# ZhongLingXiao/nano-kazen

Hardware: NVIDIA B200
Metric: Mpaths/s (higher is better)
Workload: dtype f32

## Files before the change

nano-kazen_b200/csrc/kz_kernels.cuh:

```cuda
#ifndef KZ_KERNELS_CUH
#define KZ_KERNELS_CUH
#include "kz_path.h"

#ifndef KZ_TRACE_THREADS
#define KZ_TRACE_THREADS 128
#endif
#ifndef KZ_TRACE_MIN_BLOCKS
#define KZ_TRACE_MIN_BLOCKS 8
#endif
#ifndef KZ_BATCH_MIN_BLOCKS
#define KZ_BATCH_MIN_BLOCKS 8
#endif
#define KZ_SHADE_THREADS 128

struct KzControl {
    unsigned long long ext_shadow[2];
    uint32_t n_class[KZ_NUM_CLASSES];
    uint32_t head_ext, head_shadow, head_trace;
    uint32_t pad[1];
    unsigned long long paths, rays_ext, rays_shadow, vertices, rays_seeded;
};

struct KzQueues {
    uint32_t *ext[2];
    uint32_t *cls[KZ_NUM_CLASSES];
    uint32_t *shadow;
};

struct KzChunk {
    int32_t x0, y0, x1, y1;
    uint32_t tiles_x;
    uint32_t npx_padded;
    int32_t spp_begin;
    uint32_t n_spp;
    uint32_t spp_group;
    unsigned long long first;
    uint32_t count;
};

#define KZ_FULL 0xFFFFFFFFu

__device__ __forceinline__ uint32_t kz_lane() { return threadIdx.x & 31u; }

__device__ __forceinline__ void kz_push(uint32_t *queue, uint32_t *counter, bool pred, uint32_t value) {
// ... 37 lines not shown
        v += __shfl_down_sync(KZ_FULL, v, o);
        h += __shfl_down_sync(KZ_FULL, h, o);
    }
    if (kz_lane() == 0u) {
        if (e) atomicAdd(&ctl->rays_ext, e);
        if (s) atomicAdd(&ctl->rays_shadow, s);
        if (v) atomicAdd(&ctl->vertices, v);
        if (h) atomicAdd(&ctl->rays_seeded, h);
    }
}

struct KzRayIn { float ox, oy, oz, tmin, dx, dy, dz, tmax; };
#ifndef KZ_FETCH_ND
#define KZ_FETCH_ND 0
#endif
#ifndef KZ_FETCH_NW
#define KZ_FETCH_NW 8
#endif
#ifndef KZ_TRAV_MODE
#define KZ_TRAV_MODE 0
#endif
#ifndef KZ_WAIT_IDLE
#define KZ_WAIT_IDLE 1
#endif
#ifndef KZ_POSTPONE_NUM
#define KZ_POSTPONE_NUM 1
#define KZ_POSTPONE_DEN 5
#endif

template <class Job>
__device__ __forceinline__ void kz_warp_trace(const KzScene &sc, const KzStackRef &stk, uint32_t *cursor, uint32_t n, Job &job) {
    KzTrav t;
    KzLocalStack ls;
    t.sp = 0; t.ng_y = 0u; t.tg_y = 0u;
    bool active = false, finished = false, exhausted = false;
    uint32_t item = 0u;
    const uint32_t lane = kz_lane(), lt = (1u << lane) - 1u;
    for (;;) {
        if (finished) {
            KzRayIn r;
            if (job.end(item, t.best, r)) kz_trav_init(sc, t, r.ox, r.oy, r.oz, r.dx, r.dy, r.dz, r.tmin, r.tmax);
            else active = false;
            finished = false;
        }
        if (!exhausted) {
            const uint32_t idle = __ballot_sync(KZ_FULL, !active);
            if (idle) {
                const uint32_t leader = (uint32_t)__ffs((int)idle) - 1u;
                uint32_t base = 0u;
                if (lane == leader) base = atomicAdd(cursor, (uint32_t)__popc(idle));
                base = __shfl_sync(KZ_FULL, base, (int)leader);
                if (!active) {
                    const uint32_t idx = base + (uint32_t)__popc(idle & lt);
                    if (idx < n) {
                        item = idx;
                        KzRayIn r;
                        job.begin(item, r);
                        kz_trav_init(sc, t, r.ox, r.oy, r.oz, r.dx, r.dy, r.dz, r.tmin, r.tmax);
                        job.seed(sc, t);
                        active = true;
                    }
                }
                exhausted = base + (uint32_t)__popc(idle) >= n;
            }
        }
        if (!__any_sync(KZ_FULL, active)) break;
        int lost = 0;
#if KZ_TRAV_MODE == 1
        while (active && !finished) {
            for (;;) {
                if (t.ng_y > 0x00FFFFFFu) kz_trav_node(sc, t, stk, ls);
                if (t.tg_y != 0u) break;
                if (t.ng_y <= 0x00FFFFFFu) {
                    if (t.sp == 0) break;
                    kz_trav_pop(t, stk, ls);
                }
            }
            while (t.tg_y != 0u) kz_trav_tri(sc, t);
            if (t.ng_y <= 0x00FFFFFFu) {
                if (t.sp == 0) finished = true;
                else kz_trav_pop(t, stk, ls);
            }
            if (!exhausted) {
                lost += 32 - __popc(__activemask()) - KZ_FETCH_ND;
                if (lost >= KZ_FETCH_NW) break;
            }
        }
#else
        while (active && !finished) {
#if KZ_WAIT_IDLE
            if (t.tg_y == 0u && t.ng_y > 0x00FFFFFFu) kz_trav_node(sc, t, stk, ls);
            const int total = __popc(__activemask());
// ... 59 lines not shown
    }
}

__global__ void __launch_bounds__(KZ_SHADE_THREADS) k_raygen(KzScene sc, KzPathState st, uint32_t *q0, KzChunk ch) {
    const uint32_t i = blockIdx.x * blockDim.x + threadIdx.x;
    if (i >= ch.count) return;
    unsigned long long g = ch.first + i;
    const unsigned long long per_block = (unsigned long long)ch.npx_padded * ch.spp_group;
    const uint32_t blk = (uint32_t)(g / per_block);
    g -= (unsigned long long)blk * per_block;
    const uint32_t left = ch.n_spp - blk * ch.spp_group;
    const uint32_t grp = left < ch.spp_group ? left : ch.spp_group;
    const uint32_t tile = (uint32_t)(g / (32u * grp));
    const uint32_t r = (uint32_t)(g - (unsigned long long)tile * (32u * grp));
    const uint32_t s_local = blk * ch.spp_group + (r >> 5), in_tile = r & 31u;
    const int x = ch.x0 + (int)((tile % ch.tiles_x) * 8u + (in_tile & 7u));
    const int y = ch.y0 + (int)((tile / ch.tiles_x) * 4u + (in_tile >> 3));
    if (x < ch.x1 && y < ch.y1) kz_raygen_item(sc, st, i, x, y, (uint32_t)(ch.spp_begin + (int)s_local));
    else {
        const float nan = kz_u2f(0x7FC00000u);
        KzRayRec ray; ray.o = mkf4(0.f, 0.f, 0.f, 0.f); ray.d = mkf4(nan, nan, nan, 0.f);
        st.a[i].ray = ray;
        st.b[i].smp.pix = 0xFFFFFFFFu;
    }
    q0[i] = i;
}

template <bool FIRST>
struct KzExtendJob {
    static constexpr bool kStopsEarly = false;
    __device__ __forceinline__ bool stop(const KzScene &, const KzTrav &) { return false; }
    const KzScene &sc; const KzPathState &st; KzControl *ctl; const KzQueues &q; const uint32_t *queue;
    uint2 *hint;
    KzCounters cnt;
    uint32_t slot, n_seeded;
    KzHit first_hit; bool retraced;
    kz3 d;
    __device__ KzExtendJob(const KzScene &s, const KzPathState &p, KzControl *c, const KzQueues &qq, const uint32_t *qu, uint2 *h)
        : sc(s), st(p), ctl(c), q(qq), queue(qu), hint(h), n_seeded(0u) { cnt.paths = cnt.rays_ext = cnt.rays_shadow = cnt.vertices = cnt.rays_seeded = 0ull; }
    __device__ __forceinline__ size_t hint_index() const {
        const uint32_t pix = st.b[slot].smp.pix, px = pix & 0xFFFFu, py = pix >> 16;
        if (px >= (uint32_t)sc.camera.width || py >= (uint32_t)sc.camera.height) return ~(size_t)0;
        return (size_t)py * (uint32_t)sc.camera.width + px;
    }
    __device__ __forceinline__ void seed(const KzScene &s, KzTrav &t) {
        if (!FIRST || hint == nullptr) return;
        const size_t i = hint_index();
        if (i == ~(size_t)0) return;
        const uint2 h = hint[i];
        n_seeded += kz_trav_seed(s, t, h.x, h.y) ? 1u : 0u;
    }
    __device__ __forceinline__ void begin(uint32_t item, KzRayIn &r) {
        slot = queue[item];
        const KzRayRec ray = st.a[slot].ray;
        const KzF4 ro = ray.o, rd = ray.d;
        r.ox = ro.x; r.oy = ro.y; r.oz = ro.z; r.tmin = ro.w; r.dx = rd.x; r.dy = rd.y; r.dz = rd.z; r.tmax = rd.w;
        d = mk3(rd.x, rd.y, rd.z);
        retraced = false;
    }
    __device__ __forceinline__ bool end(uint32_t, const KzHit &hit, KzRayIn &r) {
        if (FIRST && isnan(d.x)) return false;
        cnt.rays_ext += 1;
        KzHit h = hit;
        if (FIRST) {
            if (hint != nullptr && !retraced) { const size_t i = hint_index(); if (i != ~(size_t)0) hint[i] = make_uint2(h.geom, h.prim); }
            if (retraced) { if (h.geom == KZ_INVALID_ID) h = first_hit; }
            else if (h.geom != KZ_INVALID_ID && sc.integrator.type == KZ_INTEGRATOR_PATH_MIS) {
                const uint32_t fl = sc.meshes[h.geom].flags;
                if ((fl & KZ_MESH_IS_LIGHT) && !(fl & KZ_MESH_LIGHT_VISIBLE)) {
                    KzIts its; its.acc_rough = 0.f;
                    fill_intersection(sc, h, its, mk3(0.f));
                    const kz3 o = its.p + sc.integrator.trace_bias * d;
                    r.ox = o.x; r.oy = o.y; r.oz = o.z; r.tmin = KZ_EPSILON; r.dx = d.x; r.dy = d.y; r.dz = d.z; r.tmax = KZ_INF;
                    first_hit = h; retraced = true;
                    return true;
                }
            }
        }
        st.a[slot].hit = mk_hit_rec(h);
        kz_push_divergent(q.cls, ctl->n_class, kz_classify(sc, h.geom), slot);
        return false;
    }
};

template <bool FIRST>
__global__ void __launch_bounds__(KZ_TRACE_THREADS, KZ_TRACE_MIN_BLOCKS) k_extend(KzScene sc, KzPathState st, KzControl *ctl, KzQueues q, int cur, uint2 *hint) {
    const KzStackRef stk = kz_trav_shared_init();
    KzExtendJob<FIRST> job(sc, st, ctl, q, q.ext[cur], FIRST ? hint : nullptr);
    kz_warp_trace(sc, stk, &ctl->head_ext, kz_ext_count(ctl, cur), job);
    job.cnt.rays_seeded = job.n_seeded;
    kz_flush_counters(ctl, job.cnt);
}

#ifndef KZ_SHADE_BLOCK_PUSH
#define KZ_SHADE_BLOCK_PUSH 1
#endif
#ifndef KZ_SHADE_MIN_BLOCKS_DIFFUSE
#define KZ_SHADE_MIN_BLOCKS_DIFFUSE 8
#endif
#ifndef KZ_SHADE_MIN_BLOCKS_TERMINAL
#define KZ_SHADE_MIN_BLOCKS_TERMINAL 4
#endif
#ifndef KZ_SHADE_MIN_BLOCKS
#define KZ_SHADE_MIN_BLOCKS 4
#endif
template <int CLS>
__global__ void __launch_bounds__(KZ_SHADE_THREADS, (CLS == KZ_CLASS_DIFFUSE ? KZ_SHADE_MIN_BLOCKS_DIFFUSE : (CLS == KZ_CLASS_TERMINAL ? KZ_SHADE_MIN_BLOCKS_TERMINAL : KZ_SHADE_MIN_BLOCKS))) k_shade(KzScene sc, KzPathState st, KzControl *ctl, KzQueues q, int nxt, int bounce) {
    const uint32_t n = ctl->n_class[CLS];
    const uint32_t *queue = q.cls[CLS];
    const uint32_t stride = gridDim.x * blockDim.x;
    KzCounters cnt; cnt.paths = cnt.rays_ext = cnt.rays_shadow = cnt.vertices = cnt.rays_seeded = 0ull;
#if KZ_SHADE_BLOCK_PUSH
    constexpr int NW = KZ_SHADE_THREADS / 32;
    __shared__ uint32_t s_cnt[2][2][NW];
    __shared__ unsigned long long s_base[2];
    int par = 0;
    for (uint32_t bbase = blockIdx.x * blockDim.x; bbase < n; bbase += stride, par ^= 1) {
        const uint32_t idx = bbase + threadIdx.x;
        uint32_t slot = 0u, flags = 0u;
        if (idx < n) {
            slot = queue[idx];
            flags = kz_shade_item<CLS>(sc, st, slot, bounce, cnt);
        }
        if (CLS != KZ_CLASS_TERMINAL) {
// ... 3 lines not shown
            if (lane == 0u) { s_cnt[par][0][w] = (uint32_t)__popc(ma); s_cnt[par][1][w] = (uint32_t)__popc(mb); }
            __syncthreads();
            if (threadIdx.x == 0) {
                uint32_t ta = 0u, tb = 0u;
#pragma unroll
                for (int k = 0; k < NW; ++k) { ta += s_cnt[par][0][k]; tb += s_cnt[par][1][k]; }
                s_base[par] = (ta | tb) ? atomicAdd(&ctl->ext_shadow[nxt], (unsigned long long)ta | ((unsigned long long)tb << 32)) : 0ull;
            }
            __syncthreads();
            uint32_t oa = (uint32_t)(s_base[par] & 0xFFFFFFFFull), ob = (uint32_t)(s_base[par] >> 32);
#pragma unroll
            for (int k = 0; k < NW; ++k) if ((uint32_t)k < w) { oa += s_cnt[par][0][k]; ob += s_cnt[par][1][k]; }
            if (pa) q.ext[nxt][oa + (uint32_t)__popc(ma & lt)] = slot;
            if (pb) q.shadow[ob + (uint32_t)__popc(mb & lt)] = slot;
        }
    }
#else
    for (uint32_t base = (blockIdx.x * blockDim.x + threadIdx.x) & ~31u; base < n; base += stride) {
        const uint32_t idx = base + kz_lane();
        uint32_t slot = 0u, flags = 0u;
        if (idx < n) {
            slot = queue[idx];
            flags = kz_shade_item<CLS>(sc, st, slot, bounce, cnt);
        }
        __syncwarp();
        if (CLS != KZ_CLASS_TERMINAL)
            kz_push2(q.ext[nxt], q.shadow, &ctl->ext_shadow[nxt], (flags & KZ_SHADE_CONTINUE) != 0u, (flags & KZ_SHADE_SHADOW) != 0u, slot);
    }
#endif
    kz_flush_counters(ctl, cnt);
}

struct KzWalk {
    kz3 o, d; float tmax; int seg;
    __device__ __forceinline__ void start(KzRayIn &r, kz3 o_, kz3 d_, float tmin, float tmax_) {
        o = o_; d = d_; tmax = tmax_; seg = 0;
        r.ox = o.x; r.oy = o.y; r.oz = o.z; r.tmin = tmin; r.dx = d.x; r.dy = d.y; r.dz = d.z; r.tmax = tmax;
    }
    __device__ __forceinline__ static bool settles(const KzScene &sc, const KzTrav &t) {
        if (sc.integrator.type != KZ_INTEGRATOR_PATH_MIS) return true;
        const uint32_t fl = sc.meshes[t.best.geom].flags;
        if ((fl & KZ_MESH_IS_LIGHT) && !(fl & KZ_MESH_LIGHT_VISIBLE)) return false;
        return sc.n_invisible_lights == 0 || kz_trav_misses_box(t, sc.inv_light_lo, sc.inv_light_hi, t.best.t);
    }
    __device__ __forceinline__ int step(const KzScene &sc, const KzHit &h, float eps, KzRayIn &r) {
        ++seg;
        if (h.geom == KZ_INVALID_ID) return 0;
        const uint32_t fl = sc.meshes[h.geom].flags;
        if (!(fl & KZ_MESH_IS_LIGHT) || (fl & KZ_MESH_LIGHT_VISIBLE) || sc.integrator.type != KZ_INTEGRATOR_PATH_MIS) return 1;
        if (seg > 4096) return 0;
        o = o + d * (h.t + eps);
        tmax = tmax - h.t;
        r.ox = o.x; r.oy = o.y; r.oz = o.z; r.tmin = eps; r.dx = d.x; r.dy = d.y; r.dz = d.z; r.tmax = tmax;
        return 2;
    }
};
struct KzShadowJob {
    static constexpr bool kStopsEarly = true;
    __device__ __forceinline__ bool stop(const KzScene &s, const KzTrav &t) { return KzWalk::settles(s, t); }
    __device__ __forceinline__ void seed(const KzScene &, KzTrav &) {}
    const KzScene &sc; const KzPathState &st; const uint32_t *queue;
    KzCounters cnt; uint32_t slot; KzWalk walk;
    __device__ KzShadowJob(const KzScene &s, const KzPathState &p, const uint32_t *qu) : sc(s), st(p), queue(qu) { cnt.paths = cnt.rays_ext = cnt.rays_shadow = cnt.vertices = cnt.rays_seeded = 0ull; }
    __device__ __forceinline__ void begin(uint32_t item, KzRayIn &r) {
        slot = queue[item];
        const KzF4 so = st.a[slot].ray.o;
        const KzShdRec shd = st.c[slot].shd;
        walk.start(r, mk3(so.x, so.y, so.z), mk3(shd.d.x, shd.d.y, shd.d.z), shd.pending.w, shd.d.w);
    }
    __device__ __forceinline__ bool end(uint32_t, const KzHit &h, KzRayIn &r) {
        cnt.rays_shadow += 1;
        const int s = walk.step(sc, h, sc.integrator.trace_bias, r);
        if (s == 2) return true;
        if (s == 0) {
            const KzF4 p = st.c[slot].shd.pending;
            KzF4 L = st.b[slot].rad.L;
            L.x += p.x; L.y += p.y; L.z += p.z;
            st.b[slot].rad.L = L;
        }
        return false;
    }
};
__global__ void __launch_bounds__(KZ_TRACE_THREADS, KZ_TRACE_MIN_BLOCKS) k_shadow(KzScene sc, KzPathState st, KzControl *ctl, KzQueues q, int nxt) {
    const KzStackRef stk = kz_trav_shared_init();
    KzShadowJob job(sc, st, q.shadow);
    kz_warp_trace(sc, stk, &ctl->head_shadow, kz_shadow_count(ctl, nxt), job);
    kz_flush_counters(ctl, job.cnt);
}

#ifndef KZ_ACC_MAX_TEXELS
#define KZ_ACC_MAX_TEXELS 160
#endif
__global__ void __launch_bounds__(KZ_SHADE_THREADS) k_accumulate(KzScene sc, KzPathState st, uint32_t count, KzF4 *frame, int rx0, int ry0) {
    __shared__ float s_table[33];
    __shared__ KzF4 s_region[KZ_SHADE_THREADS / 32][KZ_ACC_MAX_TEXELS];
    if (threadIdx.x < 33) s_table[threadIdx.x] = sc.filter.table[threadIdx.x];
    const uint32_t lane = threadIdx.x & 31u;
    KzF4 *region = s_region[threadIdx.x >> 5];
    for (uint32_t e = lane; e < KZ_ACC_MAX_TEXELS; e += 32u) region[e] = mkf4(0.f, 0.f, 0.f, 0.f);
    __syncthreads();
    const float radius = sc.filter.radius, lookup = 32 / radius;
    const int b = sc.border, cols = sc.camera.width + 2 * b, rows = sc.camera.height + 2 * b;
    const int lo = -(int)floorf(radius + 0.5f), hi = (int)ceilf(radius + 0.5f) - 1;
    const int tw = 8 + hi - lo, th = 4 + hi - lo;
    const bool tiled = tw * th <= KZ_ACC_MAX_TEXELS;
    const uint32_t n_units = (count + 31u) >> 5, n_warps = (gridDim.x * blockDim.x) >> 5;
    const uint32_t w = (blockIdx.x * blockDim.x + threadIdx.x) >> 5, per = (n_units + n_warps - 1u) / n_warps;
    const uint32_t u1 = min(n_units, (w + 1u) * per);
    int cur_x = 0, cur_y = 0; bool open = false;
    for (uint32_t u = w * per; u < u1; ++u) {
        const uint32_t i = (u << 5) + lane;
        KzSplat sp = {};
        bool ok = i < count && st.b[i].smp.pix != 0xFFFFFFFFu && kz_splat_of(sc, st, i, sp);
        if (!tiled) { if (ok) kz_accumulate_item(sc, st, i, frame, s_table); continue; }
        if (ok && (sp.x0 < sp.ipx + b + lo || sp.x1 > sp.ipx + b + hi || sp.y0 < sp.ipy + b + lo || sp.y1 > sp.ipy + b + hi)) { kz_accumulate_item(sc, st, i, frame, s_table); ok = false; }
        const uint32_t m = __ballot_sync(KZ_FULL, ok);
        if (!m) continue;
        const int leader = __ffs((int)m) - 1;
        const int tx = __shfl_sync(KZ_FULL, ok ? rx0 + ((sp.ipx - rx0) & ~7) : 0, leader), ty = __shfl_sync(KZ_FULL, ok ? ry0 + ((sp.ipy - ry0) & ~3) : 0, leader);
        if (open && (tx != cur_x || ty != cur_y)) {
// ... 7 lines not shown
        }
        cur_x = tx; cur_y = ty; open = true;
        const int bx = ok ? sp.ipx - tx - lo : 0, by = ok ? sp.ipy - ty - lo : 0;
        for (int dy = lo; dy <= hi; ++dy) {
            const int Y = sp.ipy + b + dy;
            const bool rowok = ok && Y >= sp.y0 && Y <= sp.y1;
            const float wy = rowok ? s_table[(int)(fabsf((float)Y - sp.py) * lookup)] : 0.f;
            for (int dx = lo; dx <= hi; ++dx) {
                const int X = sp.ipx + b + dx;
                if (rowok && X >= sp.x0 && X <= sp.x1) {
                    const float wx = s_table[(int)(fabsf((float)X - sp.px) * lookup)];
                    KzF4 *p = region + ((by + dy) * tw + (bx + dx));
                    KzF4 v = *p;
                    v.x += sp.value.x * wx * wy; v.y += sp.value.y * wx * wy; v.z += sp.value.z * wx * wy; v.w += 1.0f * wx * wy;
                    *p = v;
                }
                __syncwarp();
            }
        }
    }
    if (tiled && open) {
        __syncwarp();
        for (int e = (int)lane; e < tw * th; e += 32) {
            const KzF4 v = region[e];
            const int X = cur_x + b + lo + e % tw, Y = cur_y + b + lo + e / tw;
            if ((v.x != 0.f || v.y != 0.f || v.z != 0.f || v.w != 0.f) && X >= 0 && X < cols && Y >= 0 && Y < rows) KZ_FRAME_ADD(frame + ((size_t)Y * cols + X), v.x, v.y, v.z, v.w);
        }
    }
}

struct KzTraceJob {
    static constexpr bool kStopsEarly = false;
    __device__ __forceinline__ bool stop(const KzScene &, const KzTrav &) { return false; }
    __device__ __forceinline__ void seed(const KzScene &, KzTrav &) {}
    const KzF4 *rays; float *hits;
    __device__ __forceinline__ void begin(uint32_t item, KzRayIn &r) {
        const KzU4 a = kz_load_u4(rays + 2 * (size_t)item), b = kz_load_u4(rays + 2 * (size_t)item + 1);
        r.ox = kz_u2f(a.x); r.oy = kz_u2f(a.y); r.oz = kz_u2f(a.z); r.tmin = kz_u2f(a.w);
        r.dx = kz_u2f(b.x); r.dy = kz_u2f(b.y); r.dz = kz_u2f(b.z); r.tmax = kz_u2f(b.w);
    }
    __device__ __forceinline__ bool end(uint32_t item, const KzHit &h, KzRayIn &) {
        float *o = hits + 5 * (size_t)item;
        o[0] = h.t; o[1] = h.u; o[2] = h.v; o[3] = kz_u2f(h.prim); o[4] = kz_u2f(h.geom);
        return false;
    }
};
__global__ void __launch_bounds__(KZ_TRACE_THREADS, KZ_BATCH_MIN_BLOCKS) k_trace(KzScene sc, const KzF4 *rays, uint32_t n, float *hits, uint32_t *cursor, KzControl *ctl) {
    const KzStackRef stk = kz_trav_shared_init();
    KzTraceJob job; job.rays = rays; job.hits = hits;
    kz_warp_trace(sc, stk, cursor, n, job);
    if (blockIdx.x == 0 && threadIdx.x == 0) atomicAdd(&ctl->rays_ext, (unsigned long long)n);
}

struct KzOccludedJob {
    static constexpr bool kStopsEarly = true;
    __device__ __forceinline__ bool stop(const KzScene &s, const KzTrav &t) { return KzWalk::settles(s, t); }
    __device__ __forceinline__ void seed(const KzScene &, KzTrav &) {}
    const KzScene &sc; const KzF4 *rays; float eps; uint8_t *occ, *segments;
    KzCounters cnt; KzWalk walk;
    __device__ KzOccludedJob(const KzScene &s, const KzF4 *r, float e, uint8_t *o, uint8_t *sg) : sc(s), rays(r), eps(e), occ(o), segments(sg) {
        cnt.paths = cnt.rays_ext = cnt.rays_shadow = cnt.vertices = cnt.rays_seeded = 0ull;
    }
    __device__ __forceinline__ void begin(uint32_t item, KzRayIn &r) {
        const KzU4 a = kz_load_u4(rays + 2 * (size_t)item), b = kz_load_u4(rays + 2 * (size_t)item + 1);
        walk.start(r, mk3(kz_u2f(a.x), kz_u2f(a.y), kz_u2f(a.z)), mk3(kz_u2f(b.x), kz_u2f(b.y), kz_u2f(b.z)), kz_u2f(a.w), kz_u2f(b.w));
    }
    __device__ __forceinline__ bool end(uint32_t item, const KzHit &h, KzRayIn &r) {
        cnt.rays_shadow += 1;
        const int s = walk.step(sc, h, eps, r);
        if (s == 2) return true;
        occ[item] = (uint8_t)s;
        if (segments) segments[item] = (uint8_t)(walk.seg > 255 ? 255 : walk.seg);
        return false;
    }
};
__global__ void __launch_bounds__(KZ_TRACE_THREADS, KZ_BATCH_MIN_BLOCKS) k_occluded(KzScene sc, const KzF4 *rays, uint32_t n, float eps, uint8_t *occ, uint8_t *segments,
                                                                uint32_t *cursor, KzControl *ctl) {
    const KzStackRef stk = kz_trav_shared_init();
    KzOccludedJob job(sc, rays, eps, occ, segments);
    kz_warp_trace(sc, stk, cursor, n, job);
    kz_flush_counters(ctl, job.cnt);
}

__global__ void k_sample_dump(KzScene sc, const int32_t *triples, uint32_t n, const char *pattern, uint32_t per, float *out) {
    const uint32_t i = blockIdx.x * blockDim.x + threadIdx.x;
    if (i >= n) return;
    KzSampler sm;
    kz_sampler_start(sc, sm, triples[3 * i], triples[3 * i + 1], (uint32_t)triples[3 * i + 2]);
    float *o = out + (size_t)i * per;
    for (const char *p = pattern; *p; ++p) {
        if (*p == '1') *o++ = kz_next1d(sc, sm);
        else { const kz2 v = (*p == 'P') ? kz_next_pixel2d(sc, sm) : kz_next2d(sc, sm); *o++ = v.x; *o++ = v.y; }
    }
}

__global__ void k_camera_rays(KzScene sc, const KzF4 *samples, uint32_t n, KzF4 *out) {
    const uint32_t i = blockIdx.x * blockDim.x + threadIdx.x;
    if (i >= n) return;
    const KzF4 s = samples[i];
    KzF4 ro, rd;
    kz_camera_ray(sc.camera, mk2(s.x, s.y), mk2(s.z, s.w), ro, rd);
    out[2 * (size_t)i] = ro; out[2 * (size_t)i + 1] = rd;
}

struct KzBsdfQuery { float wi[3], wo[3], uv[2], acc_rough, s1, s2[2]; int32_t mesh, mode; };
__global__ void k_bsdf_query(KzScene sc, const KzBsdfQuery *qs, uint32_t n, float *out8) {
    const uint32_t i = blockIdx.x * blockDim.x + threadIdx.x;
    if (i >= n) return;
    const KzBsdfQuery q = qs[i];
    KzIts its;
    its.sh.s = mk3(1, 0, 0); its.sh.t = mk3(0, 1, 0); its.sh.n = mk3(0, 0, 1);
    its.geo_n = its.sh.n; its.dpdu = mk3(1, 0, 0); its.uv = mk2(q.uv[0], q.uv[1]); its.mesh = q.mesh; its.acc_rough = q.acc_rough;
    its.p = mk3(0.f);
    const KzBsdfCtx bc = bsdf_ctx(sc, its);
// ... 87 lines not shown
```

nano-kazen_b200/csrc/kz_traverse.h:

```cpp
#ifndef KZ_TRAVERSE_H
#define KZ_TRAVERSE_H
#include "kz_scene.h"

struct KzHit { float t, u, v; uint32_t prim, geom; };

#if KZ_DEVICE_CODE
#define KZ_LDG_U4(ptr) __ldg(reinterpret_cast<const uint4 *>(ptr))
KZ_HD KzU4 kz_load_u4(const void *p) { uint4 v = KZ_LDG_U4(p); KzU4 r; r.x = v.x; r.y = v.y; r.z = v.z; r.w = v.w; return r; }
#else
KZ_HD KzU4 kz_load_u4(const void *p) { KzU4 r; memcpy(&r, p, 16); return r; }
#endif

KZ_HD float kz_edot(float ax, float ay, float az, float bx, float by, float bz) {
    return kz_fma(ax, bx, kz_fma(ay, by, kz_mul(az, bz)));
}
KZ_HD float kz_fms(float a, float b, float c) { return kz_fma(a, b, -c); }

KZ_HD bool kz_pluecker(float ox, float oy, float oz, float dx, float dy, float dz, float tnear, float tfar,
                       KzU4 a, KzU4 b, KzU4 c, float &t_out, float &u_out, float &v_out) {
    float v0x = kz_sub(kz_u2f(a.x), ox), v0y = kz_sub(kz_u2f(a.y), oy), v0z = kz_sub(kz_u2f(a.z), oz);
    float v1x = kz_sub(kz_u2f(b.x), ox), v1y = kz_sub(kz_u2f(b.y), oy), v1z = kz_sub(kz_u2f(b.z), oz);
    float v2x = kz_sub(kz_u2f(c.x), ox), v2y = kz_sub(kz_u2f(c.y), oy), v2z = kz_sub(kz_u2f(c.z), oz);
    float e0x = kz_sub(v2x, v0x), e0y = kz_sub(v2y, v0y), e0z = kz_sub(v2z, v0z);
    float e1x = kz_sub(v0x, v1x), e1y = kz_sub(v0y, v1y), e1z = kz_sub(v0z, v1z);
// ... 44 lines not shown
#endif
#ifndef KZ_SLACK
#define KZ_SLACK 3.814697265625e-06f
#endif
#ifndef KZ_SHORT_STACK
#define KZ_SHORT_STACK 8
#endif
#define KZ_LOCAL_STACK (64 - KZ_SHORT_STACK)
#define KZ_POSTPONE_SP_LIMIT 32
#define KZ_MAX_ACCEL_DEPTH (KZ_SHORT_STACK + KZ_LOCAL_STACK - 2 - KZ_POSTPONE_SP_LIMIT)

#ifndef KZ_TRACE_THREADS
#define KZ_TRACE_THREADS 128
#endif
struct KzStackRef {
#if defined(__CUDACC__)
    uint32_t sbase;
    uint32_t lbase;
#endif
};

KZ_HD uint32_t kz_perm8(uint32_t m, uint32_t c) {
    if (c & 1u) m = ((m & 0x55u) << 1) | ((m >> 1) & 0x55u);
    if (c & 2u) m = ((m & 0x33u) << 2) | ((m >> 2) & 0x33u);
    if (c & 4u) m = ((m & 0x0Fu) << 4) | (m >> 4);
    return m;
}
KZ_HD uint32_t kz_spread7(uint32_t m) {
    m = (m | (m << 8)) & 0x0000F00Fu;
    m = (m | (m << 4)) & 0x000C30C3u;
    m = (m | (m << 2)) & 0x00249249u;
    return m * 7u;
}
#if defined(__CUDACC__)
__shared__ uint32_t kz_s_lut[512 + 256];
__shared__ uint2    kz_s_stack[KZ_SHORT_STACK * KZ_TRACE_THREADS];
__device__ __forceinline__ KzStackRef kz_trav_shared_init() {
    uint8_t *perm = reinterpret_cast<uint8_t *>(kz_s_lut);
    for (uint32_t i = threadIdx.x; i < 8u * 256u; i += blockDim.x) perm[i] = (uint8_t)kz_perm8(i & 255u, i >> 8);
    for (uint32_t i = threadIdx.x; i < 256u; i += blockDim.x) kz_s_lut[512 + i] = kz_spread7(i);
    __syncthreads();
    KzStackRef stk;
    stk.sbase = (uint32_t)__cvta_generic_to_shared(kz_s_stack + threadIdx.x);
    stk.lbase = (uint32_t)__cvta_generic_to_shared(kz_s_lut);
    asm volatile("mov.b32 %0, %0;" : "+r"(stk.sbase));
    asm volatile("mov.b32 %0, %0;" : "+r"(stk.lbase));
    return stk;
}
__device__ __forceinline__ uint32_t kz_lds_u8(uint32_t a) { uint32_t r; asm volatile("ld.shared.u8 %0, [%1];" : "=r"(r) : "r"(a)); return r; }
__device__ __forceinline__ uint32_t kz_lds_u32(uint32_t a) { uint32_t r; asm volatile("ld.shared.u32 %0, [%1];" : "=r"(r) : "r"(a)); return r; }
#endif

struct KzTrav {
    float ox, oy, oz, dx, dy, dz, tmin;
    float rdx, rdy, rdz;
    float cnx, cny, cnz, cfx, cfy, cfz;
    uint32_t oct_inv;
    KzHit best;
    uint32_t ng_x, ng_y;
    uint32_t tg_x, tg_y, tg_m;
    int sp;
};
struct KzLocalStack { uint32_t x[KZ_LOCAL_STACK], y[KZ_LOCAL_STACK]; };

KZ_HD void kz_trav_init(const KzScene &sc, KzTrav &t, float ox, float oy, float oz, float dx, float dy, float dz, float tmin, float tmax) {
    t.ox = ox; t.oy = oy; t.oz = oz; t.dx = dx; t.dy = dy; t.dz = dz; t.tmin = tmin;
    t.best.t = tmax; t.best.u = 0.f; t.best.v = 0.f; t.best.prim = KZ_INVALID_ID; t.best.geom = KZ_INVALID_ID;
    const float slack = (fmaxf(fabsf(ox), fmaxf(fabsf(oy), fabsf(oz))) + sc.scene_max_abs) * KZ_SLACK;
    t.rdx = kz_rcp_safe(dx); t.rdy = kz_rcp_safe(dy); t.rdz = kz_rcp_safe(dz);
    const bool nx = t.rdx < 0.f, ny = t.rdy < 0.f, nz = t.rdz < 0.f;
    t.cnx = -((nx ? ox - slack : ox + slack) * t.rdx); t.cfx = -((nx ? ox + slack : ox - slack) * t.rdx);
    t.cny = -((ny ? oy - slack : oy + slack) * t.rdy); t.cfy = -((ny ? oy + slack : oy - slack) * t.rdy);
    t.cnz = -((nz ? oz - slack : oz + slack) * t.rdz); t.cfz = -((nz ? oz + slack : oz - slack) * t.rdz);
    t.oct_inv = ((nx ? 0u : 1u) | (ny ? 0u : 2u) | (nz ? 0u : 4u));
    const bool has_nan = isnan(ox) || isnan(oy) || isnan(oz) || isnan(dx) || isnan(dy) || isnan(dz) || isnan(tmin) || isnan(tmax);
    t.ng_x = 0u; t.ng_y = (sc.n_nodes && !has_nan) ? 0x80000000u : 0u;
    t.tg_x = 0u; t.tg_y = 0u; t.tg_m = 0u;
    t.sp = 0;
}

KZ_HD void kz_trav_push(KzTrav &t, const KzStackRef &stk, KzLocalStack &ls, uint32_t x, uint32_t y) {
#if KZ_DEVICE_CODE
    if (t.sp < KZ_SHORT_STACK) asm volatile("st.shared.v2.u32 [%0], {%1, %2};" :: "r"(stk.sbase + (uint32_t)t.sp * (8u * KZ_TRACE_THREADS)), "r"(x), "r"(y) : "memory");
    else { ls.x[t.sp - KZ_SHORT_STACK] = x; ls.y[t.sp - KZ_SHORT_STACK] = y; }
#else
    (void)stk; ls.x[t.sp] = x; ls.y[t.sp] = y;
#endif
    ++t.sp;
}
KZ_HD void kz_trav_pop1(KzTrav &t, const KzStackRef &stk, const KzLocalStack &ls, uint32_t &x, uint32_t &y) {
    --t.sp;
#if KZ_DEVICE_CODE
    if (t.sp < KZ_SHORT_STACK) asm volatile("ld.shared.v2.u32 {%0, %1}, [%2];" : "=r"(x), "=r"(y) : "r"(stk.sbase + (uint32_t)t.sp * (8u * KZ_TRACE_THREADS)) : "memory");
    else { x = ls.x[t.sp - KZ_SHORT_STACK]; y = ls.y[t.sp - KZ_SHORT_STACK]; }
#else
    (void)stk; x = ls.x[t.sp]; y = ls.y[t.sp];
#endif
}
KZ_HD void kz_trav_pop(KzTrav &t, const KzStackRef &stk, const KzLocalStack &ls) {
    kz_trav_pop1(t, stk, ls, t.ng_x, t.ng_y);
    if (t.ng_y <= 0x00FFFFFFu) {
        uint32_t unused;
        t.tg_x = t.ng_x; t.tg_y = t.ng_y; t.ng_x = 0u; t.ng_y = 0u;
        kz_trav_pop1(t, stk, ls, t.tg_m, unused);
    }
}
KZ_HD void kz_trav_postpone(KzTrav &t, const KzStackRef &stk, KzLocalStack &ls) {
    kz_trav_push(t, stk, ls, t.tg_m, 0u);
    kz_trav_push(t, stk, ls, t.tg_x, t.tg_y);
    t.tg_y = 0u;
}

// ... 51 lines not shown
#undef KZ_Q2F
#undef KZ_Q2M
    }
    const uint32_t hit8 = ~miss & 0xFFu;
#if KZ_DEVICE_CODE
    const uint32_t hi = kz_lds_u8(stk.lbase + (t.oct_inv << 8) + (hit8 & imask));
    const uint32_t sp7 = kz_lds_u32(stk.lbase + 2048u + (hit8 << 2));
#else
    const uint32_t hi = kz_perm8(hit8 & imask, t.oct_inv);
    const uint32_t sp7 = kz_spread7(hit8);
#endif
    t.ng_x = n1.x;
    t.ng_y = (hi << 24) | imask;
    t.tg_x = n1.y;
    t.tg_m = n1.z;
    t.tg_y = sp7 & n1.z;
}

KZ_HD bool kz_trav_misses_box(const KzTrav &t, const float *lo, const float *hi, float tfar) {
    const bool nx = !(t.oct_inv & 1u), ny = !(t.oct_inv & 2u), nz = !(t.oct_inv & 4u);
    const float tnx = fmaf(nx ? hi[0] : lo[0], t.rdx, t.cnx), tfx = fmaf(nx ? lo[0] : hi[0], t.rdx, t.cfx);
    const float tny = fmaf(ny ? hi[1] : lo[1], t.rdy, t.cny), tfy = fmaf(ny ? lo[1] : hi[1], t.rdy, t.cfy);
    const float tnz = fmaf(nz ? hi[2] : lo[2], t.rdz, t.cnz), tfz = fmaf(nz ? lo[2] : hi[2], t.rdz, t.cfz);
    const float cmin = fmaxf(fmaxf(tnx, tny), fmaxf(tnz, t.tmin));
    const float cmax = fminf(fminf(tfx, tfy), fminf(tfz, tfar));
    return cmin > cmax;
}

KZ_HD bool kz_trav_tri(const KzScene &sc, KzTrav &t) {
    const uint32_t ti = kz_bfind(t.tg_y);
    t.tg_y &= ~(1u << ti);
    const KzF4 *tp = sc.tris + (size_t)(t.tg_x + kz_popc(t.tg_m & ~(0xFFFFFFFFu << ti))) * 3;
    const KzU4 a = kz_load_u4(tp), b = kz_load_u4(tp + 1), c = kz_load_u4(tp + 2);
    float tt, u, v;
    if (kz_pluecker(t.ox, t.oy, t.oz, t.dx, t.dy, t.dz, t.tmin, t.best.t, a, b, c, tt, u, v)) {
        const uint32_t geom = a.w, prim = b.w;
        const bool better = tt < t.best.t || geom < t.best.geom || (geom == t.best.geom && prim < t.best.prim);
        if (better) { t.best.t = tt; t.best.u = u; t.best.v = v; t.best.geom = geom; t.best.prim = prim; }
        return better;
    }
    return false;
}

KZ_HD bool kz_trav_seed(const KzScene &sc, KzTrav &t, uint32_t geom, uint32_t prim) {
    if (geom >= sc.n_meshes || t.ng_y == 0u) return false;
    const KzMeshRec &m = sc.meshes[geom];
    if (prim >= m.n_triangles) return false;
    const KzU4 ix = kz_load_u4(sc.indices + (m.index_offset + prim));
    const KzVertex *vb = sc.vertices + m.vertex_offset;
    const KzU4 a = kz_load_u4(vb + ix.x), b = kz_load_u4(vb + ix.y), c = kz_load_u4(vb + ix.z);
    float tt, u, v;
    if (!kz_pluecker(t.ox, t.oy, t.oz, t.dx, t.dy, t.dz, t.tmin, t.best.t, a, b, c, tt, u, v)) return false;
    t.best.t = tt; t.best.u = u; t.best.v = v; t.best.geom = geom; t.best.prim = prim;
    return true;
}

KZ_HD KzHit kz_trace(const KzScene &sc, const KzStackRef &stk, float ox, float oy, float oz, float dx, float dy, float dz,
                     float tmin, float tmax, bool any_hit, uint32_t seed_geom = KZ_INVALID_ID, uint32_t seed_prim = KZ_INVALID_ID) {
    KzTrav t;
    KzLocalStack ls;
    kz_trav_init(sc, t, ox, oy, oz, dx, dy, dz, tmin, tmax);
    if (sc.n_nodes == 0) return t.best;
    if (!any_hit) kz_trav_seed(sc, t, seed_geom, seed_prim);
    for (;;) {
        if (t.ng_y > 0x00FFFFFFu) kz_trav_node(sc, t, stk, ls);
        while (t.tg_y != 0u) {
            kz_trav_tri(sc, t);
            if (any_hit && t.best.geom != KZ_INVALID_ID) return t.best;
        }
        if (t.ng_y <= 0x00FFFFFFu) {
            if (t.sp == 0) break;
            kz_trav_pop(t, stk, ls);
        }
    }
    return t.best;
}

#endif
```

Baseline: 980.6.

## Spill ray origin, direction and hit payload to shared memory to cut registers

Result: faster. 991.5 (median of 6 runs) (+1.1%).

```diff
diff --git a/nano-kazen_b200/csrc/kz_kernels.cuh b/nano-kazen_b200/csrc/kz_kernels.cuh
--- a/nano-kazen_b200/csrc/kz_kernels.cuh
+++ b/nano-kazen_b200/csrc/kz_kernels.cuh
@@ -9,7 +9,7 @@
 #define KZ_TRACE_MIN_BLOCKS 8
 #endif
 #ifndef KZ_BATCH_MIN_BLOCKS
-#define KZ_BATCH_MIN_BLOCKS 8
+#define KZ_BATCH_MIN_BLOCKS 9
 #endif
 #define KZ_SHADE_THREADS 128
 
@@ -113,6 +113,7 @@
 __device__ __forceinline__ void kz_warp_trace(const KzScene &sc, const KzStackRef &stk, uint32_t *cursor, uint32_t n, Job &job) {
     KzTrav t;
     KzLocalStack ls;
+    kz_trav_bind(t, stk);
     t.sp = 0; t.ng_y = 0u; t.tg_y = 0u;
     bool active = false, finished = false, exhausted = false;
     uint32_t item = 0u;
@@ -120,7 +121,7 @@
     for (;;) {
         if (finished) {
             KzRayIn r;
-            if (job.end(item, t.best, r)) kz_trav_init(sc, t, r.ox, r.oy, r.oz, r.dx, r.dy, r.dz, r.tmin, r.tmax);
+            if (job.end(item, t, r)) kz_trav_init(sc, t, r.ox, r.oy, r.oz, r.dx, r.dy, r.dz, r.tmin, r.tmax);
             else active = false;
             finished = false;
         }
@@ -138,7 +139,7 @@
                         KzRayIn r;
                         job.begin(item, r);
                         kz_trav_init(sc, t, r.ox, r.oy, r.oz, r.dx, r.dy, r.dz, r.tmin, r.tmax);
-                        job.seed(sc, t);
+                        job.start(sc, t);
                         active = true;
                     }
                 }
@@ -264,19 +265,18 @@
     __device__ __forceinline__ bool stop(const KzScene &, const KzTrav &) { return false; }
     const KzScene &sc; const KzPathState &st; KzControl *ctl; const KzQueues &q; const uint32_t *queue;
     uint2 *hint;
-    KzCounters cnt;
-    uint32_t slot, n_seeded;
-    KzHit first_hit; bool retraced;
-    kz3 d;
+    uint32_t slot, n_rays, n_seeded;
     __device__ KzExtendJob(const KzScene &s, const KzPathState &p, KzControl *c, const KzQueues &qq, const uint32_t *qu, uint2 *h)
-        : sc(s), st(p), ctl(c), q(qq), queue(qu), hint(h), n_seeded(0u) { cnt.paths = cnt.rays_ext = cnt.rays_shadow = cnt.vertices = cnt.rays_seeded = 0ull; }
+        : sc(s), st(p), ctl(c), q(qq), queue(qu), hint(h), n_rays(0u), n_seeded(0u) {}
     __device__ __forceinline__ size_t hint_index() const {
         const uint32_t pix = st.b[slot].smp.pix, px = pix & 0xFFFFu, py = pix >> 16;
         if (px >= (uint32_t)sc.camera.width || py >= (uint32_t)sc.camera.height) return ~(size_t)0;
         return (size_t)py * (uint32_t)sc.camera.width + px;
     }
-    __device__ __forceinline__ void seed(const KzScene &s, KzTrav &t) {
-        if (!FIRST || hint == nullptr) return;
+    __device__ __forceinline__ void start(const KzScene &s, KzTrav &t) {
+        if (!FIRST) return;
+        kz_trav_set_job_word(t, 0u);
+        if (hint == nullptr) return;
         const size_t i = hint_index();
         if (i == ~(size_t)0) return;
         const uint2 h = hint[i];
@@ -287,16 +287,21 @@
         const KzRayRec ray = st.a[slot].ray;
         const KzF4 ro = ray.o, rd = ray.d;
         r.ox = ro.x; r.oy = ro.y; r.oz = ro.z; r.tmin = ro.w; r.dx = rd.x; r.dy = rd.y; r.dz = rd.z; r.tmax = rd.w;
-        d = mk3(rd.x, rd.y, rd.z);
-        retraced = false;
-    }
-    __device__ __forceinline__ bool end(uint32_t, const KzHit &hit, KzRayIn &r) {
+    }
+    __device__ __forceinline__ bool end(uint32_t, KzTrav &t, KzRayIn &r) {
+        const kz3 d = kz_trav_dir(t);
         if (FIRST && isnan(d.x)) return false;
-        cnt.rays_ext += 1;
-        KzHit h = hit;
+        n_rays += 1u;
+        KzHit h = kz_trav_hit(t);
         if (FIRST) {
+            const bool retraced = kz_trav_job_word(t) != 0u;
             if (hint != nullptr && !retraced) { const size_t i = hint_index(); if (i != ~(size_t)0) hint[i] = make_uint2(h.geom, h.prim); }
-            if (retraced) { if (h.geom == KZ_INVALID_ID) h = first_hit; }
+            if (retraced) {
+                if (h.geom == KZ_INVALID_ID) {
+                    const KzHitRec f = st.a[slot].hit;
+                    h.t = f.t; h.u = f.u; h.v = f.v; h.prim = f.prim; h.geom = f.geom;
+                }
+            }
             else if (h.geom != KZ_INVALID_ID && sc.integrator.type == KZ_INTEGRATOR_PATH_MIS) {
                 const uint32_t fl = sc.meshes[h.geom].flags;
                 if ((fl & KZ_MESH_IS_LIGHT) && !(fl & KZ_MESH_LIGHT_VISIBLE)) {
@@ -304,7 +309,8 @@
                     fill_intersection(sc, h, its, mk3(0.f));
                     const kz3 o = its.p + sc.integrator.trace_bias * d;
                     r.ox = o.x; r.oy = o.y; r.oz = o.z; r.tmin = KZ_EPSILON; r.dx = d.x; r.dy = d.y; r.dz = d.z; r.tmax = KZ_INF;
-                    first_hit = h; retraced = true;
+                    st.a[slot].hit = mk_hit_rec(h);
+                    kz_trav_set_job_word(t, 1u);
                     return true;
                 }
             }
@@ -320,8 +326,9 @@
     const KzStackRef stk = kz_trav_shared_init();
     KzExtendJob<FIRST> job(sc, st, ctl, q, q.ext[cur], FIRST ? hint : nullptr);
     kz_warp_trace(sc, stk, &ctl->head_ext, kz_ext_count(ctl, cur), job);
-    job.cnt.rays_seeded = job.n_seeded;
-    kz_flush_counters(ctl, job.cnt);
+    KzCounters cnt = {};
+    cnt.rays_ext = job.n_rays; cnt.rays_seeded = job.n_seeded;
+    kz_flush_counters(ctl, cnt);
 }
 
 #ifndef KZ_SHADE_BLOCK_PUSH
@@ -391,23 +398,26 @@
 }
 
 struct KzWalk {
-    kz3 o, d; float tmax; int seg;
-    __device__ __forceinline__ void start(KzRayIn &r, kz3 o_, kz3 d_, float tmin, float tmax_) {
-        o = o_; d = d_; tmax = tmax_; seg = 0;
+    float tmax; int seg;
+    __device__ __forceinline__ void start(KzRayIn &r, kz3 o, kz3 d, float tmin, float tmax_) {
+        tmax = tmax_; seg = 0;
         r.ox = o.x; r.oy = o.y; r.oz = o.z; r.tmin = tmin; r.dx = d.x; r.dy = d.y; r.dz = d.z; r.tmax = tmax;
     }
     __device__ __forceinline__ static bool settles(const KzScene &sc, const KzTrav &t) {
         if (sc.integrator.type != KZ_INTEGRATOR_PATH_MIS) return true;
-        const uint32_t fl = sc.meshes[t.best.geom].flags;
+        const uint32_t fl = sc.meshes[kz_trav_hit_geom(t)].flags;
         if ((fl & KZ_MESH_IS_LIGHT) && !(fl & KZ_MESH_LIGHT_VISIBLE)) return false;
         return sc.n_invisible_lights == 0 || kz_trav_misses_box(t, sc.inv_light_lo, sc.inv_light_hi, t.best.t);
     }
-    __device__ __forceinline__ int step(const KzScene &sc, const KzHit &h, float eps, KzRayIn &r) {
+    __device__ __forceinline__ int step(const KzScene &sc, const KzTrav &t, float eps, KzRayIn &r) {
         ++seg;
+        const KzHit h = kz_trav_hit(t);
         if (h.geom == KZ_INVALID_ID) return 0;
         const uint32_t fl = sc.meshes[h.geom].flags;
         if (!(fl & KZ_MESH_IS_LIGHT) || (fl & KZ_MESH_LIGHT_VISIBLE) || sc.integrator.type != KZ_INTEGRATOR_PATH_MIS) return 1;
         if (seg > 4096) return 0;
+        kz3 o, d;
+        kz_trav_ray(t, o, d);
         o = o + d * (h.t + eps);
         tmax = tmax - h.t;
         r.ox = o.x; r.oy = o.y; r.oz = o.z; r.tmin = eps; r.dx = d.x; r.dy = d.y; r.dz = d.z; r.tmax = tmax;
@@ -417,19 +427,19 @@
 struct KzShadowJob {
     static constexpr bool kStopsEarly = true;
     __device__ __forceinline__ bool stop(const KzScene &s, const KzTrav &t) { return KzWalk::settles(s, t); }
-    __device__ __forceinline__ void seed(const KzScene &, KzTrav &) {}
+    __device__ __forceinline__ void start(const KzScene &, KzTrav &) {}
     const KzScene &sc; const KzPathState &st; const uint32_t *queue;
-    KzCounters cnt; uint32_t slot; KzWalk walk;
-    __device__ KzShadowJob(const KzScene &s, const KzPathState &p, const uint32_t *qu) : sc(s), st(p), queue(qu) { cnt.paths = cnt.rays_ext = cnt.rays_shadow = cnt.vertices = cnt.rays_seeded = 0ull; }
+    uint32_t n_rays, slot; KzWalk walk;
+    __device__ KzShadowJob(const KzScene &s, const KzPathState &p, const uint32_t *qu) : sc(s), st(p), queue(qu), n_rays(0u) {}
     __device__ __forceinline__ void begin(uint32_t item, KzRayIn &r) {
         slot = queue[item];
         const KzF4 so = st.a[slot].ray.o;
         const KzShdRec shd = st.c[slot].shd;
         walk.start(r, mk3(so.x, so.y, so.z), mk3(shd.d.x, shd.d.y, shd.d.z), shd.pending.w, shd.d.w);
     }
-    __device__ __forceinline__ bool end(uint32_t, const KzHit &h, KzRayIn &r) {
-        cnt.rays_shadow += 1;
-        const int s = walk.step(sc, h, sc.integrator.trace_bias, r);
+    __device__ __forceinline__ bool end(uint32_t, KzTrav &t, KzRayIn &r) {
+        n_rays += 1u;
+        const int s = walk.step(sc, t, sc.integrator.trace_bias, r);
         if (s == 2) return true;
         if (s == 0) {
             const KzF4 p = st.c[slot].shd.pending;
@@ -444,7 +454,9 @@
     const KzStackRef stk = kz_trav_shared_init();
     KzShadowJob job(sc, st, q.shadow);
     kz_warp_trace(sc, stk, &ctl->head_shadow, kz_shadow_count(ctl, nxt), job);
-    kz_flush_counters(ctl, job.cnt);
+    KzCounters cnt = {};
+    cnt.rays_shadow = job.n_rays;
+    kz_flush_counters(ctl, cnt);
 }
 
 #ifndef KZ_ACC_MAX_TEXELS
@@ -518,14 +530,15 @@
 struct KzTraceJob {
     static constexpr bool kStopsEarly = false;
     __device__ __forceinline__ bool stop(const KzScene &, const KzTrav &) { return false; }
-    __device__ __forceinline__ void seed(const KzScene &, KzTrav &) {}
+    __device__ __forceinline__ void start(const KzScene &, KzTrav &) {}
     const KzF4 *rays; float *hits;
     __device__ __forceinline__ void begin(uint32_t item, KzRayIn &r) {
         const KzU4 a = kz_load_u4(rays + 2 * (size_t)item), b = kz_load_u4(rays + 2 * (size_t)item + 1);
         r.ox = kz_u2f(a.x); r.oy = kz_u2f(a.y); r.oz = kz_u2f(a.z); r.tmin = kz_u2f(a.w);
         r.dx = kz_u2f(b.x); r.dy = kz_u2f(b.y); r.dz = kz_u2f(b.z); r.tmax = kz_u2f(b.w);
     }
-    __device__ __forceinline__ bool end(uint32_t item, const KzHit &h, KzRayIn &) {
+    __device__ __forceinline__ bool end(uint32_t item, KzTrav &t, KzRayIn &) {
+        const KzHit h = kz_trav_hit(t);
         float *o = hits + 5 * (size_t)item;
         o[0] = h.t; o[1] = h.u; o[2] = h.v; o[3] = kz_u2f(h.prim); o[4] = kz_u2f(h.geom);
         return false;
@@ -541,19 +554,17 @@
 struct KzOccludedJob {
     static constexpr bool kStopsEarly = true;
     __device__ __forceinline__ bool stop(const KzScene &s, const KzTrav &t) { return KzWalk::settles(s, t); }
-    __device__ __forceinline__ void seed(const KzScene &, KzTrav &) {}
+    __device__ __forceinline__ void start(const KzScene &, KzTrav &) {}
     const KzScene &sc; const KzF4 *rays; float eps; uint8_t *occ, *segments;
-    KzCounters cnt; KzWalk walk;
-    __device__ KzOccludedJob(const KzScene &s, const KzF4 *r, float e, uint8_t *o, uint8_t *sg) : sc(s), rays(r), eps(e), occ(o), segments(sg) {
-        cnt.paths = cnt.rays_ext = cnt.rays_shadow = cnt.vertices = cnt.rays_seeded = 0ull;
-    }
+    uint32_t n_rays; KzWalk walk;
+    __device__ KzOccludedJob(const KzScene &s, const KzF4 *r, float e, uint8_t *o, uint8_t *sg) : sc(s), rays(r), eps(e), occ(o), segments(sg), n_rays(0u) {}
     __device__ __forceinline__ void begin(uint32_t item, KzRayIn &r) {
         const KzU4 a = kz_load_u4(rays + 2 * (size_t)item), b = kz_load_u4(rays + 2 * (size_t)item + 1);
         walk.start(r, mk3(kz_u2f(a.x), kz_u2f(a.y), kz_u2f(a.z)), mk3(kz_u2f(b.x), kz_u2f(b.y), kz_u2f(b.z)), kz_u2f(a.w), kz_u2f(b.w));
     }
-    __device__ __forceinline__ bool end(uint32_t item, const KzHit &h, KzRayIn &r) {
-        cnt.rays_shadow += 1;
-        const int s = walk.step(sc, h, eps, r);
+    __device__ __forceinline__ bool end(uint32_t item, KzTrav &t, KzRayIn &r) {
+        n_rays += 1u;
+        const int s = walk.step(sc, t, eps, r);
         if (s == 2) return true;
         occ[item] = (uint8_t)s;
         if (segments) segments[item] = (uint8_t)(walk.seg > 255 ? 255 : walk.seg);
@@ -565,7 +576,9 @@
     const KzStackRef stk = kz_trav_shared_init();
     KzOccludedJob job(sc, rays, eps, occ, segments);
     kz_warp_trace(sc, stk, cursor, n, job);
-    kz_flush_counters(ctl, job.cnt);
+    KzCounters cnt = {};
+    cnt.rays_shadow = job.n_rays;
+    kz_flush_counters(ctl, cnt);
 }
 
 __global__ void k_sample_dump(KzScene sc, const int32_t *triples, uint32_t n, const char *pattern, uint32_t per, float *out) {
diff --git a/nano-kazen_b200/csrc/kz_traverse.h b/nano-kazen_b200/csrc/kz_traverse.h
--- a/nano-kazen_b200/csrc/kz_traverse.h
+++ b/nano-kazen_b200/csrc/kz_traverse.h
@@ -100,9 +100,10 @@
     m = (m | (m << 2)) & 0x00249249u;
     return m * 7u;
 }
+#define KZ_RAY_PAIRS 6
 #if defined(__CUDACC__)
 __shared__ uint32_t kz_s_lut[512 + 256];
-__shared__ uint2    kz_s_stack[KZ_SHORT_STACK * KZ_TRACE_THREADS];
+__shared__ uint2    kz_s_stack[(KZ_SHORT_STACK + KZ_RAY_PAIRS) * KZ_TRACE_THREADS];
 __device__ __forceinline__ KzStackRef kz_trav_shared_init() {
     uint8_t *perm = reinterpret_cast<uint8_t *>(kz_s_lut);
     for (uint32_t i = threadIdx.x; i < 8u * 256u; i += blockDim.x) perm[i] = (uint8_t)kz_perm8(i & 255u, i >> 8);
@@ -117,23 +118,123 @@
 }
 __device__ __forceinline__ uint32_t kz_lds_u8(uint32_t a) { uint32_t r; asm volatile("ld.shared.u8 %0, [%1];" : "=r"(r) : "r"(a)); return r; }
 __device__ __forceinline__ uint32_t kz_lds_u32(uint32_t a) { uint32_t r; asm volatile("ld.shared.u32 %0, [%1];" : "=r"(r) : "r"(a)); return r; }
-#endif
-
+__device__ __forceinline__ void kz_sts2(uint32_t a, uint32_t x, uint32_t y) { asm volatile("st.shared.v2.u32 [%0], {%1, %2};" :: "r"(a), "r"(x), "r"(y)); }
+__device__ __forceinline__ void kz_lds2(uint32_t a, uint32_t &x, uint32_t &y) { asm volatile("ld.shared.v2.u32 {%0, %1}, [%2];" : "=r"(x), "=r"(y) : "r"(a)); }
+#endif
+
+#if KZ_DEVICE_CODE
+struct KzTravBest { float t; };
+#else
+typedef KzHit KzTravBest;
+#endif
 struct KzTrav {
-    float ox, oy, oz, dx, dy, dz, tmin;
+#if KZ_DEVICE_CODE
+    uint32_t rec;
+#else
+    float ox, oy, oz, dx, dy, dz;
+    uint32_t job;
+#endif
+    float tmin;
     float rdx, rdy, rdz;
     float cnx, cny, cnz, cfx, cfy, cfz;
     uint32_t oct_inv;
-    KzHit best;
+    KzTravBest best;
     uint32_t ng_x, ng_y;
     uint32_t tg_x, tg_y, tg_m;
     int sp;
 };
 struct KzLocalStack { uint32_t x[KZ_LOCAL_STACK], y[KZ_LOCAL_STACK]; };
 
+KZ_HD void kz_trav_bind(KzTrav &t, const KzStackRef &stk) {
+#if KZ_DEVICE_CODE
+    t.rec = stk.sbase + KZ_SHORT_STACK * 8u * KZ_TRACE_THREADS;
+#else
+    (void)t; (void)stk;
+#endif
+}
+#if KZ_DEVICE_CODE
+#define KZ_REC(k) (t.rec + (k) * 8u * KZ_TRACE_THREADS)
+#endif
+KZ_HD kz3 kz_trav_org(const KzTrav &t) {
+#if KZ_DEVICE_CODE
+    uint32_t a, b, c, unused;
+    kz_lds2(KZ_REC(0), a, b); kz_lds2(KZ_REC(1), c, unused);
+    return mk3(kz_u2f(a), kz_u2f(b), kz_u2f(c));
+#else
+    return mk3(t.ox, t.oy, t.oz);
+#endif
+}
+KZ_HD kz3 kz_trav_dir(const KzTrav &t) {
+#if KZ_DEVICE_CODE
+    uint32_t a, b, c, unused;
+    kz_lds2(KZ_REC(1), unused, a); kz_lds2(KZ_REC(2), b, c);
+    return mk3(kz_u2f(a), kz_u2f(b), kz_u2f(c));
+#else
+    return mk3(t.dx, t.dy, t.dz);
+#endif
+}
+KZ_HD void kz_trav_ray(const KzTrav &t, kz3 &o, kz3 &d) {
+#if KZ_DEVICE_CODE
+    uint32_t a, b, c, e, f, g;
+    kz_lds2(KZ_REC(0), a, b); kz_lds2(KZ_REC(1), c, e); kz_lds2(KZ_REC(2), f, g);
+    o = mk3(kz_u2f(a), kz_u2f(b), kz_u2f(c)); d = mk3(kz_u2f(e), kz_u2f(f), kz_u2f(g));
+#else
+    o = mk3(t.ox, t.oy, t.oz); d = mk3(t.dx, t.dy, t.dz);
+#endif
+}
+KZ_HD void kz_trav_set_best(KzTrav &t, float tt, float u, float v, uint32_t prim, uint32_t geom) {
+    t.best.t = tt;
+#if KZ_DEVICE_CODE
+    kz_sts2(KZ_REC(3), kz_f2u(u), kz_f2u(v)); kz_sts2(KZ_REC(4), prim, geom);
+#else
+    t.best.u = u; t.best.v = v; t.best.prim = prim; t.best.geom = geom;
+#endif
+}
+KZ_HD uint32_t kz_trav_hit_geom(const KzTrav &t) {
+#if KZ_DEVICE_CODE
+    uint32_t prim, geom;
+    kz_lds2(KZ_REC(4), prim, geom);
+    return geom;
+#else
+    return t.best.geom;
+#endif
+}
+KZ_HD KzHit kz_trav_hit(const KzTrav &t) {
+#if KZ_DEVICE_CODE
+    KzHit h; uint32_t u, v;
+    h.t = t.best.t;
+    kz_lds2(KZ_REC(3), u, v); kz_lds2(KZ_REC(4), h.prim, h.geom);
+    h.u = kz_u2f(u); h.v = kz_u2f(v);
+    return h;
+#else
+    return t.best;
+#endif
+}
+KZ_HD uint32_t kz_trav_job_word(const KzTrav &t) {
+#if KZ_DEVICE_CODE
+    uint32_t w, unused;
+    kz_lds2(KZ_REC(5), w, unused);
+    return w;
+#else
+    return t.job;
+#endif
+}
+KZ_HD void kz_trav_set_job_word(KzTrav &t, uint32_t w) {
+#if KZ_DEVICE_CODE
+    kz_sts2(KZ_REC(5), w, 0u);
+#else
+    t.job = w;
+#endif
+}
+
 KZ_HD void kz_trav_init(const KzScene &sc, KzTrav &t, float ox, float oy, float oz, float dx, float dy, float dz, float tmin, float tmax) {
-    t.ox = ox; t.oy = oy; t.oz = oz; t.dx = dx; t.dy = dy; t.dz = dz; t.tmin = tmin;
-    t.best.t = tmax; t.best.u = 0.f; t.best.v = 0.f; t.best.prim = KZ_INVALID_ID; t.best.geom = KZ_INVALID_ID;
+#if KZ_DEVICE_CODE
+    kz_sts2(KZ_REC(0), kz_f2u(ox), kz_f2u(oy)); kz_sts2(KZ_REC(1), kz_f2u(oz), kz_f2u(dx)); kz_sts2(KZ_REC(2), kz_f2u(dy), kz_f2u(dz));
+#else
+    t.ox = ox; t.oy = oy; t.oz = oz; t.dx = dx; t.dy = dy; t.dz = dz;
+#endif
+    t.tmin = tmin;
+    kz_trav_set_best(t, tmax, 0.f, 0.f, KZ_INVALID_ID, KZ_INVALID_ID);
     const float slack = (fmaxf(fabsf(ox), fmaxf(fabsf(oy), fabsf(oz))) + sc.scene_max_abs) * KZ_SLACK;
     t.rdx = kz_rcp_safe(dx); t.rdy = kz_rcp_safe(dy); t.rdz = kz_rcp_safe(dz);
     const bool nx = t.rdx < 0.f, ny = t.rdy < 0.f, nz = t.rdz < 0.f;
@@ -146,6 +247,7 @@
     t.tg_x = 0u; t.tg_y = 0u; t.tg_m = 0u;
     t.sp = 0;
 }
+#undef KZ_REC
 
 KZ_HD void kz_trav_push(KzTrav &t, const KzStackRef &stk, KzLocalStack &ls, uint32_t x, uint32_t y) {
 #if KZ_DEVICE_CODE
@@ -263,11 +365,17 @@
     t.tg_y &= ~(1u << ti);
     const KzF4 *tp = sc.tris + (size_t)(t.tg_x + kz_popc(t.tg_m & ~(0xFFFFFFFFu << ti))) * 3;
     const KzU4 a = kz_load_u4(tp), b = kz_load_u4(tp + 1), c = kz_load_u4(tp + 2);
+    kz3 o, d;
+    kz_trav_ray(t, o, d);
     float tt, u, v;
-    if (kz_pluecker(t.ox, t.oy, t.oz, t.dx, t.dy, t.dz, t.tmin, t.best.t, a, b, c, tt, u, v)) {
+    if (kz_pluecker(o.x, o.y, o.z, d.x, d.y, d.z, t.tmin, t.best.t, a, b, c, tt, u, v)) {
         const uint32_t geom = a.w, prim = b.w;
-        const bool better = tt < t.best.t || geom < t.best.geom || (geom == t.best.geom && prim < t.best.prim);
-        if (better) { t.best.t = tt; t.best.u = u; t.best.v = v; t.best.geom = geom; t.best.prim = prim; }
+        bool better = tt < t.best.t;
+        if (!better) {
+            const KzHit h = kz_trav_hit(t);
+            better = geom < h.geom || (geom == h.geom && prim < h.prim);
+        }
+        if (better) kz_trav_set_best(t, tt, u, v, prim, geom);
         return better;
     }
     return false;
@@ -280,9 +388,11 @@
     const KzU4 ix = kz_load_u4(sc.indices + (m.index_offset + prim));
     const KzVertex *vb = sc.vertices + m.vertex_offset;
     const KzU4 a = kz_load_u4(vb + ix.x), b = kz_load_u4(vb + ix.y), c = kz_load_u4(vb + ix.z);
+    kz3 o, d;
+    kz_trav_ray(t, o, d);
     float tt, u, v;
-    if (!kz_pluecker(t.ox, t.oy, t.oz, t.dx, t.dy, t.dz, t.tmin, t.best.t, a, b, c, tt, u, v)) return false;
-    t.best.t = tt; t.best.u = u; t.best.v = v; t.best.geom = geom; t.best.prim = prim;
+    if (!kz_pluecker(o.x, o.y, o.z, d.x, d.y, d.z, t.tmin, t.best.t, a, b, c, tt, u, v)) return false;
+    kz_trav_set_best(t, tt, u, v, prim, geom);
     return true;
 }
 
@@ -290,21 +400,21 @@
                      float tmin, float tmax, bool any_hit, uint32_t seed_geom = KZ_INVALID_ID, uint32_t seed_prim = KZ_INVALID_ID) {
     KzTrav t;
     KzLocalStack ls;
+    kz_trav_bind(t, stk);
     kz_trav_init(sc, t, ox, oy, oz, dx, dy, dz, tmin, tmax);
-    if (sc.n_nodes == 0) return t.best;
+    if (sc.n_nodes == 0) return kz_trav_hit(t);
     if (!any_hit) kz_trav_seed(sc, t, seed_geom, seed_prim);
     for (;;) {
         if (t.ng_y > 0x00FFFFFFu) kz_trav_node(sc, t, stk, ls);
         while (t.tg_y != 0u) {
-            kz_trav_tri(sc, t);
-            if (any_hit && t.best.geom != KZ_INVALID_ID) return t.best;
+            if (kz_trav_tri(sc, t) && any_hit) return kz_trav_hit(t);
         }
         if (t.ng_y <= 0x00FFFFFFu) {
             if (t.sp == 0) break;
             kz_trav_pop(t, stk, ls);
         }
     }
-    return t.best;
-}
-
-#endif
+    return kz_trav_hit(t);
+}
+
+#endif
```
